# multiplefish/VPLines-SLAM

Hardware: AMD Instinct MI355X
Metric: sliding-window BA solves/sec (10 KF, 200 pts + 80 lines, 5 iters) (higher is better)
Workload: dtype f64

## Files before the change

### vplines-slam_amd/csrc/ba_step.h

```cpp
#pragma once
#include "ba_common.h"
#include "ba_solve.h"

namespace vpl {

constexpr int SCHUR_THREADS = 256;
constexpr int CHOL_THREADS = 256;
constexpr int BACK_THREADS = 256;

__device__ __forceinline__ void lds_ticket_wait(int* t, int seq) {
  while (__hip_atomic_load(t, __ATOMIC_RELAXED, __HIP_MEMORY_SCOPE_WORKGROUP) != seq) __builtin_amdgcn_s_sleep(1);
  __builtin_amdgcn_fence(__ATOMIC_ACQUIRE, "workgroup", "local");
}
__device__ __forceinline__ void lds_ticket_pass(int* t, int seq, int lane) {
  __builtin_amdgcn_fence(__ATOMIC_RELEASE, "workgroup", "local");
  if (lane == 0) __hip_atomic_store(t, seq + 1, __ATOMIC_RELAXED, __HIP_MEMORY_SCOPE_WORKGROUP);
}

__device__ __forceinline__ int compact2vis(int c, int s, int WS) {
  if (c < WS - 6) { const int v = 6 * s + c; return v < 66 ? v : -1; }
  if (c < WS) return 66 + (c - (WS - 6));
  return c < WS + 2 ? 72 + (c - WS) : -1;
}

// ... 253 lines not shown
        const int e = (h0 + u) * T + tid;
        code[u] = (h0 + u < NB && e < NZ_N) ? B.nz_tab[e] : -1;
      }
#pragma unroll
      for (int u = 0; u < HALF; ++u) hh[u] = code[u] >= 0 ? Hcc[code[u] & 0x3fff] : 0.0;
#pragma unroll
      for (int u = 0; u < HALF; ++u)
        if (code[u] >= 0) {
          const int r = (code[u] >> 14) & 255, c = code[u] >> 22;
          qq += (r == c ? 1.0 : 2.0) * uc[r] * hh[u] * uc[c];
        }
    }
  }
  VPL_STAMP(B, w, 1);
  for (int p = tid; p < nP; p += T) {
    const double s = kP[4 * p], d = kP[4 * p + 1], g = kP[4 * p + 2], h = kP[4 * p + 3];
    const double Al = s * s * h + mu * d * d;
    if (!(Al > 0.0)) flag[0] = 1;
    const double smv = s / sqrt(Al);
    pS[p] = smv;
    pE[p] = (s * g / d) / smv;
    pG[p] = smv * (g * d / s);
  }
  for (int l = tid; l < nL; l += T) {
    double Hl[16], s4[4], d4[4], g4[4];
#pragma unroll
    for (int a = 0; a < 4; ++a) { s4[a] = kL[28 * l + a]; d4[a] = kL[28 * l + 4 + a]; g4[a] = kL[28 * l + 8 + a]; }
#pragma unroll
    for (int k = 0; k < 16; ++k) Hl[k] = kL[28 * l + 12 + k];
    double A[10];
    int t = 0;
#pragma unroll
    for (int a = 0; a < 4; ++a)
#pragma unroll
      for (int b = 0; b < 4; ++b) if (b <= a) {
        A[t] = s4[a] * s4[b] * Hl[4 * a + b];
        if (a == b) A[t] += mu * d4[a] * d4[a];
        ++t;
      }
    bool ok = true;
    chol4(A, ok);
    if (!ok) flag[0] = 1;
    double us[4];
#pragma unroll
    for (int k = 0; k < 10; ++k) { lch[l * 10 + k] = A[k]; lC[l * 10 + k] = A[k]; }
#pragma unroll
    for (int a = 0; a < 4; ++a) {
      const double rd = 1.0 / A[tri(a, a)];
      lS[4 * l + a] = s4[a] * rd;
      us[a] = g4[a] / d4[a];
#pragma unroll
      for (int qd = 0; qd < 4; ++qd) if (qd < a) lC[l * 10 + tri(a, qd)] = A[tri(a, qd)] * rd;
    }
#pragma unroll
    for (int a = 0; a < 4; ++a) {
      double s2 = 0;
#pragma unroll
      for (int qd = 0; qd < 4; ++qd) if (qd >= a) s2 += A[tri(qd, a)] * us[qd];
      lE[4 * l + a] = s2;
    }
    {
      double xg[4];
#pragma unroll
      for (int a = 0; a < 4; ++a) {
        double s2 = (s4[a] / A[tri(a, a)]) * (g4[a] * d4[a] / s4[a]);
#pragma unroll
        for (int qd = 0; qd < 4; ++qd) if (qd < a) s2 -= (A[tri(a, qd)] / A[tri(a, a)]) * xg[qd];
        xg[a] = s2;
        lG[4 * l + a] = s2;
      }
    }
  }
  __syncthreads();
  for (int i = tid; i < CSQ_N; i += T) Cacc[i] = 0.0;
  for (int i = tid; i < NLT * 4 * 64; i += T) {
    const int ln = i & 63, v = (i >> 6) & 3, t = i >> 8;
    int ta = 0, tb = 0;
    tri_decode(t, ta, tb);
    const int ca = 16 * ta + (ln >> 4) + 4 * v, cb = 16 * tb + (ln & 15);
    int code = -1;
    if (ca >= cb && ca < WSv + 2 && cb < WSv) {
      const int a0 = compact2vis(ca, 0, WSv), b0 = compact2vis(cb, 0, WSv);
      const int step = (ca < WSv - 6 ? CSQ_LD : 0) + (cb < WSv - 6 ? 1 : 0);
      code = (a0 * CSQ_LD + b0) | step << 16;
    }
    ftab[i] = code;
  }
  __syncthreads();
  VPL_STAMP(B, w, 2);
  {
    const int m = lane & 15, kk = lane >> 4;
    const int wrow = lane < SK_WSTRIDE ? B.sk_wave[((size_t)w * 8 + wv) * SK_WSTRIDE + lane] : -1;
    const int nchunk = __builtin_amdgcn_readlane(wrow, 0);
    auto fetch = [&](int k) {
      int4 e = etab[k];
      e.x = __builtin_amdgcn_readfirstlane(e.x); e.y = __builtin_amdgcn_readfirstlane(e.y); e.z = __builtin_amdgcn_readfirstlane(e.z);
      return e;
    };
    v4d acc[NLT];
#pragma unroll
    for (int t = 0; t < NLT; ++t) acc[t] = v4d{0, 0, 0, 0};
    const double* Wp = B.Wp + (size_t)w * B.maxP * WS;
    const double* Wl = B.Wl + (size_t)w * B.maxL * 4 * WS;
    const double* gpv = B.gp + (size_t)w * B.maxP;
    const double* glv = B.gl + (size_t)w * B.maxL * 4;
    double wm[NTC], gm[NTC], em[NTC];
    int cl[NTC];
#pragma unroll
    for (int t = 0; t < NTC; ++t) {
      const int c = 16 * t + m;
      wm[t] = c < WSv ? 1.0 : 0.0;
      gm[t] = c == WSv ? 1.0 : 0.0;
      em[t] = c == WSv + 1 ? 1.0 : 0.0;
      cl[t] = c < WSv - 6 ? c : (c < WSv ? c + coff : WS - 1);
    }
    auto lm_id = [&](const int4 e) { return ((kk & 2 ? e.z : e.y) >> (16 * (kk & 1))) & 0xffff; };
    auto load_raw = [&](const int4 e, double (&raw)[NTC][4]) {
      const bool isl = (e.x & 32) != 0;
      const int idr = lm_id(e);
      const int id = idr != 0xffff ? idr : 0;
      if (isl) {
        const double* Wr = Wl + (unsigned)(id * 4 * WS);
#pragma unroll
        for (int t = 0; t < NTC; ++t)
#pragma unroll
          for (int qd = 0; qd < 4; ++qd) raw[t][qd] = Wr[(unsigned)(qd * WS + cl[t])];
      } else {
#pragma unroll
        for (int t = 0; t < NTC; ++t) raw[t][0] = Wp[(unsigned)(id * WS + cl[t])];
#pragma unroll
        for (int t = 0; t < NTC; ++t)
#pragma unroll
          for (int qd = 1; qd < 4; ++qd) raw[t][qd] = 0.0;
      }
    };
    auto transform = [&](const int4 e, const double (&raw)[NTC][4], double (&x)[NTC][4]) {
      const bool isl = (e.x & 32) != 0;
      const int idr = lm_id(e);
      const int id = idr != 0xffff ? idr : 0;
      const double pm = idr != 0xffff ? 1.0 : 0.0;
      if (isl) {
        const double* C = lC + id * 10;
        const double s0 = lS[4 * id] * pm, s1 = lS[4 * id + 1] * pm, s2 = lS[4 * id + 2] * pm, s3 = lS[4 * id + 3] * pm;
        const double c10 = C[1], c20 = C[3], c21 = C[4], c30 = C[6], c31 = C[7], c32 = C[8];
        double ev[4], gv[4];
#pragma unroll
        for (int a = 0; a < 4; ++a) { ev[a] = lE[4 * id + a] * pm; gv[a] = lG[4 * id + a] * pm; }
#pragma unroll
        for (int t = 0; t < NTC; ++t) {
          const double x0 = s0 * raw[t][0];
          const double x1 = s1 * raw[t][1] - c10 * x0;
          const double x2 = s2 * raw[t][2] - c20 * x0 - c21 * x1;
          const double x3 = s3 * raw[t][3] - c30 * x0 - c31 * x1 - c32 * x2;
          x[t][0] = x0 * wm[t] + gv[0] * gm[t] + ev[0] * em[t];
          x[t][1] = x1 * wm[t] + gv[1] * gm[t] + ev[1] * em[t];
          x[t][2] = x2 * wm[t] + gv[2] * gm[t] + ev[2] * em[t];
          x[t][3] = x3 * wm[t] + gv[3] * gm[t] + ev[3] * em[t];
        }
      } else {
        const double sp = pS[id] * pm, ep = pE[id] * pm, gq = pG[id] * pm;
#pragma unroll
        for (int t = 0; t < NTC; ++t) {
          x[t][0] = sp * raw[t][0] * wm[t] + gq * gm[t] + ep * em[t];
          x[t][1] = 0.0; x[t][2] = 0.0; x[t][3] = 0.0;
        }
      }
    };
#ifdef VPL_STAMPS
    long long st_flush = 0, st_wait = 0, st_xf = 0, st_mf = 0, st_ld = 0;
#endif
    auto flush = [&](int g, int seq) {
#ifdef VPL_STAMPS
      const long long tf0 = __builtin_readcyclecounter();
#endif
      const int s6 = 6 * (g & 15);
      int code[NLT * 4];
#pragma unroll
      for (int i = 0; i < NLT * 4; ++i) code[i] = ftab[i * 64 + lane];
      lds_ticket_wait(&tick[0], seq);
#ifdef VPL_STAMPS
      st_wait += __builtin_readcyclecounter() - tf0;
#endif
#pragma unroll
      for (int t = 0; t < NLT; ++t) {
        const double vals[4] = {acc[t].x, acc[t].y, acc[t].z, acc[t].w};
#pragma unroll
        for (int v = 0; v < 4; ++v) {
          const int c2 = code[4 * t + v];
          if (c2 >= 0) lds_add(&Cacc[(c2 & 0xffff) + s6 * (c2 >> 16)], vals[v]);
        }
        acc[t] = v4d{0, 0, 0, 0};
      }
      lds_ticket_pass(&tick[0], seq, lane);
#ifdef VPL_STAMPS
      st_flush += __builtin_readcyclecounter() - tf0;
#endif
    };
    int nent = 0;
#pragma unroll 1
    for (int ch = 0; ch < nchunk; ++ch) {
      const int k0 = __builtin_amdgcn_readlane(wrow, __builtin_amdgcn_readfirstlane(1 + 3 * ch));
      const int k1 = __builtin_amdgcn_readlane(wrow, __builtin_amdgcn_readfirstlane(2 + 3 * ch));
      const int seq = __builtin_amdgcn_readlane(wrow, __builtin_amdgcn_readfirstlane(3 + 3 * ch));
      nent += k1 - k0;
      if (MIXED && (fetch(k0).x & 64)) {
        SchurWide A;
        A.etab = etab; A.Wp = Wp; A.Wl = Wl; A.WS = WS; A.lC = lC; A.lS = lS; A.lE = lE; A.lG = lG; A.pS = pS; A.pE = pE; A.pG = pG;
        A.Cacc = Cacc; A.tick = tick;
        schur_wide_chunk(A, k0, k1, seq);
        continue;
      }
      double raw0[NTC][4], raw1[NTC][4], raw2[NTC][4];
      constexpr int NPF = 3;
      load_raw(fetch(k0), raw0);
      load_raw(fetch(min(k0 + 1, k1 - 1)), raw1);
      load_raw(fetch(min(k0 + 2, k1 - 1)), raw2);
      const int gcur = fetch(k0).x;
      auto step = [&](int k, double (&rw)[NTC][4]) {
        const int4 e = fetch(k);
#ifdef VPL_STAMPS
        const long long ts0 = __builtin_readcyclecounter();
#endif
        double x[NTC][4];
        transform(e, rw, x);
#ifdef VPL_STAMPS
        const long long ts1 = __builtin_readcyclecounter();
        st_xf += ts1 - ts0;
#endif
        load_raw(fetch(min(k + NPF, k1 - 1)), rw);
#ifdef VPL_STAMPS
        const long long ts2 = __builtin_readcyclecounter();
        st_ld += ts2 - ts1;
#endif
        const bool isl = (e.x & 32) != 0;
#pragma unroll
        for (int a = 0; a < 4; ++a) {
          if (a == 0 || isl) {
            int t = 0;
#pragma unroll
            for (int ta = 0; ta < NTC; ++ta)
#pragma unroll
              for (int tb = 0; tb <= ta; ++tb, ++t) acc[t] = __builtin_amdgcn_mfma_f64_16x16x4f64(x[ta][a], x[tb][a], acc[t], 0, 0, 0);
          }
        }
#ifdef VPL_STAMPS
        st_mf += __builtin_readcyclecounter() - ts2;
#endif
      };
#pragma unroll 1
      for (int kb = k0; kb < k1; kb += NPF) {
        step(kb, raw0);
        if (kb + 1 < k1) step(kb + 1, raw1);
        if (kb + 2 < k1) step(kb + 2, raw2);
      }
      flush(gcur, seq);
    }
#ifdef VPL_STAMPS
    if (lane == 0 && wv < 2) {
      long long* dg_ = B.dbg + (size_t)w * 64 + 30 + 6 * wv;
      dg_[0] = st_xf; dg_[1] = st_ld; dg_[2] = st_mf; dg_[3] = st_flush; dg_[4] = st_wait; dg_[5] = nent;
    }
#endif
  }
  __syncthreads();
  VPL_STAMP(B, w, 3);
  for (int b = tid; b < NV; b += T) qq += 2.0 * Cacc[(NV + 1) * CSQ_LD + b] * uc[vis2cam(b)];
  double* sacc = B.sacc + (size_t)w * SACC_N;
  for (int i = tid; i < SACC_N; i += T) {
    int a, b;
    tri_decode(i, a, b);
    sacc[i] = Cacc[a * CSQ_LD + b];
  }
  a1 = block_sum(a1, red);
  q = block_sum(q, red);
  qq = block_sum(qq, red);
  if (tid == 0) {
    tr->a1 = a1;
    tr->alpha = a1 / (q + qq);
    if (flag[0]) B.path[w] = 2;
  }
  VPL_STAMP(B, w, 4);
}

template <int NTC>
__global__ __launch_bounds__(SCHUR_THREADS, 2) void k_schur(DevBatch B) {
  extern __shared__ double sm[];
  if (blockIdx.x == 0 && threadIdx.x == 0) { B.ord_cnt[2 * ((B.ord_it + 1) & 1)] = 0; B.ord_cnt[2 * ((B.ord_it + 1) & 1) + 1] = 0; }
  schur_body<NTC>(B, ordered_window(B), sm);
}
__global__ __launch_bounds__(SCHUR_THREADS, 2) void k_schur_mixed(DevBatch B) {
  extern __shared__ double sm[];
  if (blockIdx.x == 0 && threadIdx.x == 0) { B.ord_cnt[2 * ((B.ord_it + 1) & 1)] = 0; B.ord_cnt[2 * ((B.ord_it + 1) & 1) + 1] = 0; }
  schur_body<3, true>(B, ordered_window(B), sm);
}
inline size_t schur_smem(int maxP, int maxL, int ntc = 5) {
  const int r1 = std::max(4 * maxP + 28 * maxL, (int)CSQ_N);
  const int maxKS = maxP / 4 + maxL + NF + 2;
  return (size_t)(r1 + 3 * maxP + 22 * maxL + 176 + 24) * sizeof(double) + (size_t)(8 + 4 * maxKS + ntc * (ntc + 1) / 2 * 256) * sizeof(int);
}

constexpr int DN = 90;
constexpr int DNT = 6;
constexpr int DNAP = DNT * (DNT + 1) / 2 * 256;
#ifdef VPL_CHOL_OCC3
constexpr int XLD = 66;
constexpr int CHOL_MIN_WAVES = 3;
#else
constexpr int XLD = 72;
constexpr int CHOL_MIN_WAVES = 2;
#endif
constexpr int XROWS_A = 36, XROWS_B = 48;

__device__ __forceinline__ int chain_frame(int ch, int b) { return ch == 0 ? 1 + b : 10 - b; }
__device__ __forceinline__ int chain_col(int ch, int b, int lane) {
  if (lane < 18) {
    const int ds = (b & 1) ? 9 : 0;
    const int f = chain_frame(ch, b);
    const int fr = (lane >= ds && lane < ds + 9) ? f : (ch == 0 ? f + 1 : f - 1);
    return 15 * fr + 6 + (lane < 9 ? lane : lane - 9);
  }
  if (ch == 0) {
    if (lane < 27) return 6 + (lane - 18);
    if (lane < 63) return 15 * ((lane - 27) / 6) + (lane - 27) % 6;
    return NC;
  }
  if (lane < 54) return 15 * (5 + (lane - 18) / 6) + (lane - 18) % 6;
  return lane == 54 ? NC : -1;
}
__device__ __forceinline__ int cam2dense(int c) {
  if (c < 0) return -1;
  if (c == NC) return DN;
  const int v = cam2vis(c);
  if (v >= 0) return v;
  if (c < 15) return 72 + (c - 6);
  return (c >= 81 && c < 90) ? c : -1;
}
__device__ __forceinline__ int dense2cam(int d) { return d < NV ? vis2cam(d) : (d < 81 ? 6 + (d - 72) : d); }
__device__ __forceinline__ int chain_dense(int ch, int lane) {
  if (lane < 18) {
    const bool s5 = ch == 0 ? lane < 9 : lane >= 9;
    return s5 ? 81 + (lane < 9 ? lane : lane - 9) : -1;
  }
  return cam2dense(chain_col(ch, 0, lane));
}

__device__ __forceinline__ void chol_body(const DevBatch& B, const int w, double* sm) {
  const int tid = threadIdx.x, T = CHOL_THREADS;
  const int lane = tid & 63, wv = ((tid >> 6) + ((blockIdx.x >> 8) & 1) * 2) & 3;
  TrState* tr = &B.tr[w];
  if (tr->status != 0 || tr->reuse != 0 || B.path[w] != 0) return;
  count_active(B, 1);
  constexpr int REG = (XROWS_A + XROWS_B) * XLD > DNAP ? (XROWS_A + XROWS_B) * XLD : DNAP;
  double* XA = sm;
  double* XBm = sm + XROWS_A * XLD;
  double* S = sm;
  double* scv = sm + REG;
  double* dgv = scv + 176;
  double* ycam = dgv + 176;
  double* yv = ycam + 176;
  double* isd = yv + 96;
  double* Linv = isd + 96;
  double* red = Linv + 256;
  int* flag = (int*)(red + 24);
  int* cdmap = flag + 8;
  double* rsL = (double*)(cdmap + 128);

  const size_t fb = (size_t)w * B.nfull;
  const double* gscale = B.scale + fb;
  const double* gdiag = B.diag + fb;
  const double* ggrad = B.grad + fb;
  double* ggn = B.gn + fb;
  const double* Hcc = B.Hcc + (size_t)w * NCP;
  const double* gc = B.gc + (size_t)w * NC;
  const double* sacc = B.sacc + (size_t)w * SACC_N;
  const double mu = tr->mu;
  for (int c = tid; c < 176; c += T) { scv[c] = c < NC ? gscale[c] : 0.0; dgv[c] = c < NC ? gdiag[c] : 1.0; ycam[c] = 0.0; }
  if (tid < 4) flag[tid] = 0;
  if (tid < 128) cdmap[tid] = chain_dense(tid >> 6, tid & 63);
  for (int i = tid; i < 3 * XLD; i += T) XBm[(XROWS_B - 3) * XLD + i] = 0.0;
  __syncthreads();
  VPL_STAMP(B, w, 8);

  double U[45];
#pragma unroll
  for (int i = 0; i < 45; ++i) U[i] = 0.0;
#define Xs(b, k) U[9 * (b) + (k)]
  if (wv < 2) {
    const int ch = wv, nblk = ch == 0 ? 4 : 5;
    double* Xout = ch == 0 ? XA : XBm;
    bool bad = false;
    auto load_strip = [&](int b, double (&raw)[9]) {
      const int col = chain_col(ch, b, lane);
      const int f = chain_frame(ch, b);
#pragma unroll
      for (int i = 0; i < 9; ++i) {
        const int r = 15 * f + 6 + i;
        raw[i] = 0.0;
        if (col == NC) raw[i] = gc[r];
        else if (col >= 0) raw[i] = Hcc[col > r ? tri(col, r) : tri(r, col)];
      }
    };
    double rawn[9];
    load_strip(0, rawn);
#pragma unroll
    for (int b = 0; b < 5; ++b) {
      if (b < nblk) {
        const int ds = (b & 1) ? 9 : 0, ns = 9 - ds;
        const int col = chain_col(ch, b, lane);
        const int f = chain_frame(ch, b);
        double R[9];
        {
          const double scol = col == NC ? 1.0 : (col >= 0 ? scv[col] : 0.0);
#pragma unroll
          for (int i = 0; i < 9; ++i) {
            const int r = 15 * f + 6 + i;
            R[i] = rawn[i] * (scv[r] * scol);
            if (col == r) R[i] += mu * dgv[r] * dgv[r];
          }
        }
        if (b + 1 < nblk) load_strip(b + 1, rawn);
        if (b > 0) {
          const bool fresh = lane >= ns && lane < ns + 9;
#pragma unroll
          for (int k = 0; k < 9; ++k) {
            const double xk = fresh ? 0.0 : Xs(b - 1, k);
#pragma unroll
            for (int i = 0; i < 9; ++i) R[i] -= readlane_f64(Xs(b - 1, k), ds + i) * xk;
          }
        }
        double piv[9];
#pragma unroll
        for (int k = 0; k < 9; ++k) {
          const double pk = readlane_f64(R[k], ds + k);
          piv[k] = pk;
          if (!(pk > 0.0)) bad = true;
          double rinv = __builtin_amdgcn_rcp(pk);
          rinv = fma(rinv, fma(-pk, rinv, 1.0), rinv);
          rinv = fma(rinv, fma(-pk, rinv, 1.0), rinv);
          const double fj = R[k] * rinv;
#pragma unroll
          for (int i = k + 1; i < 9; ++i) R[i] -= readlane_f64(R[i], ds + k) * fj;
        }
        const bool dcol = cam2dense(col) >= 0;
#pragma unroll
        for (int k = 0; k < 9; ++k) {
          double rs = __builtin_amdgcn_rsq(piv[k]);
          rs = rs * fma(-0.5 * piv[k] * rs, rs, 1.5);
          rs = rs * fma(-0.5 * piv[k] * rs, rs, 1.5);
          if (lane == 0) rsL[(5 * ch + b) * 9 + k] = rs;
          const double xv = R[k] * rs;
          Xs(b, k) = col >= 0 ? xv : 0.0;
          Xout[(9 * b + k) * XLD + lane] = dcol ? xv : 0.0;
        }
        __builtin_amdgcn_fence(__ATOMIC_RELEASE, "workgroup");
        if (lane == 0) __hip_atomic_store(&flag[1 + ch], b + 1, __ATOMIC_RELAXED, __HIP_MEMORY_SCOPE_WORKGROUP);
      }
    }
    if (bad && lane == 0) flag[0] = 1;
  } else {
    const int ch = wv - 2, nblk = ch == 0 ? 4 : 5;
    const double* Xin = ch == 0 ? XA : XBm;
    const int m = lane & 15, kk = lane >> 4;
    const int nks = (ch == 0 ? XROWS_A : XROWS_B) / 4;
    int have = 0;
    v4d pacc[10];
#pragma unroll
    for (int t = 0; t < 10; ++t) pacc[t] = v4d{0, 0, 0, 0};
    for (int ks = 0; ks < nks; ++ks) {
      const int need = min(nblk, (4 * ks + 3) / 9 + 1);
      while (have < need) {
        have = __hip_atomic_load(&flag[1 + ch], __ATOMIC_RELAXED, __HIP_MEMORY_SCOPE_WORKGROUP);
        if (have >= need) __builtin_amdgcn_fence(__ATOMIC_ACQUIRE, "workgroup");
      }
      const double* row = Xin + (4 * ks + kk) * XLD + m;
      const double x0 = row[0], x1 = row[16], x2 = row[32], x3 = row[48];
      pacc[0] = __builtin_amdgcn_mfma_f64_16x16x4f64(x0, x0, pacc[0], 0, 0, 0);
      pacc[1] = __builtin_amdgcn_mfma_f64_16x16x4f64(x1, x0, pacc[1], 0, 0, 0);
      pacc[2] = __builtin_amdgcn_mfma_f64_16x16x4f64(x1, x1, pacc[2], 0, 0, 0);
      pacc[3] = __builtin_amdgcn_mfma_f64_16x16x4f64(x2, x0, pacc[3], 0, 0, 0);
      pacc[4] = __builtin_amdgcn_mfma_f64_16x16x4f64(x2, x1, pacc[4], 0, 0, 0);
      pacc[5] = __builtin_amdgcn_mfma_f64_16x16x4f64(x2, x2, pacc[5], 0, 0, 0);
      pacc[6] = __builtin_amdgcn_mfma_f64_16x16x4f64(x3, x0, pacc[6], 0, 0, 0);
      pacc[7] = __builtin_amdgcn_mfma_f64_16x16x4f64(x3, x1, pacc[7], 0, 0, 0);
      pacc[8] = __builtin_amdgcn_mfma_f64_16x16x4f64(x3, x2, pacc[8], 0, 0, 0);
      pacc[9] = __builtin_amdgcn_mfma_f64_16x16x4f64(x3, x3, pacc[9], 0, 0, 0);
    }
#pragma unroll
    for (int t = 0; t < 10; ++t) { U[4 * t] = pacc[t].x; U[4 * t + 1] = pacc[t].y; U[4 * t + 2] = pacc[t].z; U[4 * t + 3] = pacc[t].w; }
  }
  __syncthreads();
  VPL_STAMP(B, w, 9);

  auto put = [&](int r, int c, double v) {
    S[tix(r, c)] = v;
    if ((r >> 4) == (c >> 4) && r != c) S[tix(c, r)] = v;
  };
  {
    constexpr int NVP = NV * (NV + 1) / 2;
    constexpr int NB1 = (NVP + CHOL_THREADS - 1) / CHOL_THREADS;
    constexpr int NB2 = (19 * 96 + CHOL_THREADS - 1) / CHOL_THREADS;
    double hh[NB1], ss[NB1], h2[NB2], s2[NB2];
    int rc1[NB1], rc2[NB2];
#pragma unroll
    for (int u = 0; u < NB1; ++u) {
      const int e = u * T + tid;
      hh[u] = 0.0; ss[u] = 0.0; rc1[u] = -1;
      if (e < NVP) {
        int vr, vc;
        tri_decode(e, vr, vc);
        rc1[u] = vr | vc << 8;
        hh[u] = Hcc[tri(vis2cam(vr), vis2cam(vc))];
        ss[u] = sacc[e];
      }
    }
#pragma unroll
    for (int u = 0; u < NB2; ++u) {
      const int idx = u * T + tid;
      const int i = idx / 96, dc = idx - 96 * i;
      const int dr = 72 + i;
      h2[u] = 0.0; s2[u] = 0.0; rc2[u] = -1;
      if (idx < 19 * 96 && dc <= dr && dc < DN) {
        rc2[u] = dr | dc << 8;
        const int c = dense2cam(dc);
        if (dr < DN) {
          const int r = dense2cam(dr);
          h2[u] = Hcc[r >= c ? tri(r, c) : tri(c, r)];
        } else {
          h2[u] = gc[c];
          if (dc < NV) s2[u] = sacc[tri(NV, dc)];
        }
      }
    }
    for (int i = tid; i < DNAP; i += T) S[i] = 0.0;
    __syncthreads();
    VPL_STAMP(B, w, 14);
#pragma unroll
    for (int u = 0; u < NB1; ++u)
      if (rc1[u] >= 0) {
        const int vr = rc1[u] & 255, vc = rc1[u] >> 8;
        const int r = vis2cam(vr), c = vis2cam(vc);
        double v = (hh[u] - ss[u]) * (scv[r] * scv[c]);
        if (r == c) v += mu * dgv[r] * dgv[r];
        put(vr, vc, v);
      }
#pragma unroll
    for (int u = 0; u < NB2; ++u)
      if (rc2[u] >= 0) {
        const int dr = rc2[u] & 255, dc = rc2[u] >> 8;
        const int c = dense2cam(dc);
        if (dr < DN) {
          const int r = dense2cam(dr);
          double v = h2[u] * (scv[r] * scv[c]);
          if (r == c) v += mu * dgv[r] * dgv[r];
          put(dr, dc, v);
        } else {
          put(DN, dc, (h2[u] - s2[u]) * scv[c]);
        }
      }
    if (tid < 6) S[tix(DN + tid, DN + tid)] = 1.0;
  }
  __syncthreads();
  VPL_STAMP(B, w, 15);
  auto in_both = [](int d) { return (d >= 30 && d < 36) || d >= 81; };
#pragma unroll 1
  for (int pass = 0; pass < 2; ++pass) {
    if ((wv == 2 && pass == 0) || wv == 3) {
      const int ch = wv - 2;
      const int m = lane & 15, kk = lane >> 4;
      int t = 0;
#pragma unroll
      for (int ta = 0; ta < 4; ++ta)
#pragma unroll
        for (int tb = 0; tb <= ta; ++tb, ++t) {
          const int j = 16 * tb + m, dj = cdmap[64 * ch + j];
#pragma unroll
          for (int v = 0; v < 4; ++v) {
            const int i = 16 * ta + kk + 4 * v;
            if (i < j) continue;
            const int di = cdmap[64 * ch + i];
            if (di < 0 || dj < 0) continue;
            if (ch == 1 && (in_both(di) && in_both(dj)) != (pass == 1)) continue;
            const int r = di > dj ? di : dj, c = di > dj ? dj : di;
            if (c >= DN) continue;
            const double val = U[4 * t + v];
            S[tix(r, c)] -= val;
            if ((r >> 4) == (c >> 4) && r != c) S[tix(c, r)] -= val;
          }
        }
    }
    __syncthreads();
  }
  VPL_STAMP(B, w, 10);

  {
    constexpr int NWV = CHOL_THREADS / 64;
    for (int K = 0; K < DNT; ++K) {
      auto rank_update = [&](int col, int I, int J0, int J1) {
        const int m = lane & 15, kk = lane >> 4;
        double* Ct = S + ((I * (I + 1) / 2 + col) << 8);
        v4d c;
        c.x = Ct[tsw(kk, m)]; c.y = Ct[tsw(kk + 4, m)]; c.z = Ct[tsw(kk + 8, m)]; c.w = Ct[tsw(kk + 12, m)];
        for (int J = J0; J < J1; ++J) {
          const double* Ai = S + ((I * (I + 1) / 2 + J) << 8);
          const double* Bk = S + ((col * (col + 1) / 2 + J) << 8);
#pragma unroll
          for (int ks = 0; ks < 4; ++ks) {
            const double av = -Ai[tsw(m, 4 * ks + kk)];
            const double bv = Bk[tsw(m, 4 * ks + kk)];
            c = __builtin_amdgcn_mfma_f64_16x16x4f64(av, bv, c, 0, 0, 0);
          }
        }
        Ct[tsw(kk, m)] = c.x; Ct[tsw(kk + 4, m)] = c.y; Ct[tsw(kk + 8, m)] = c.z; Ct[tsw(kk + 12, m)] = c.w;
      };
      if (wv == 0) {
        double* D = S + ((K * (K + 1) / 2 + K) << 8);
        const int r4 = lane >> 4, cc = lane & 15;
        double d[4], mm[4];
#pragma unroll
        for (int v = 0; v < 4; ++v) { d[v] = D[tsw(r4 + 4 * v, cc)]; mm[v] = (r4 + 4 * v == cc) ? 1.0 : 0.0; }
        const int ncol = min(16, DN - 16 * K);
        double pivc = 1.0;
        bool bad = false;
#define VPL_DSTEP(J) diag_tile_step<J>(d, mm, r4, cc, ncol, pivc, bad);
        VPL_DSTEP(0) VPL_DSTEP(1) VPL_DSTEP(2) VPL_DSTEP(3) VPL_DSTEP(4) VPL_DSTEP(5) VPL_DSTEP(6) VPL_DSTEP(7)
        VPL_DSTEP(8) VPL_DSTEP(9) VPL_DSTEP(10) VPL_DSTEP(11) VPL_DSTEP(12) VPL_DSTEP(13) VPL_DSTEP(14) VPL_DSTEP(15)
#undef VPL_DSTEP
        if (bad) {
          if (lane == 0) flag[0] = 1;
        } else {
          const double sq = sqrt(pivc);
          if (cc < ncol) {
#pragma unroll
            for (int v = 0; v < 4; ++v) {
              const int r = r4 + 4 * v;
              if (r > cc) D[tsw(r, cc)] = d[v] / sq;
              else if (r == cc) { const double id = 1.0 / sq; isd[16 * K + cc] = id; D[tsw(r, cc)] = 1.0 / id; }
            }
          }
          if (K < DNT - 1) {
            const double isq = 1.0 / sq;
#pragma unroll
            for (int v = 0; v < 4; ++v) {
              const int r = r4 + 4 * v;
              const double ir = __shfl(isq, r, 64);
              Linv[tsw(r, cc)] = cc <= r ? mm[v] * ir : 0.0;
            }
          }
        }
      } else if (K >= 1) {
        for (int I = K + 1 + (wv - 1); I < DNT; I += NWV - 1) rank_update(K, I, K - 1, K);
        if (K + 1 < DNT)
          for (int I = K + 1 + (wv - 1); I < DNT; I += NWV - 1) rank_update(K + 1, I, 0, K);
      }
      __syncthreads();
      if (flag[0]) break;
      for (int I = K + 1 + wv; I < DNT; I += NWV) {
        const int m = lane & 15, kk = lane >> 4;
        double* At = S + ((I * (I + 1) / 2 + K) << 8);
        v4d c = {0.0, 0.0, 0.0, 0.0};
        double av[4], bv[4];
#pragma unroll
        for (int ks = 0; ks < 4; ++ks) { av[ks] = At[tsw(m, 4 * ks + kk)]; bv[ks] = Linv[tsw(m, 4 * ks + kk)]; }
#pragma unroll
        for (int ks = 0; ks < 4; ++ks) c = __builtin_amdgcn_mfma_f64_16x16x4f64(av[ks], bv[ks], c, 0, 0, 0);
        At[tsw(kk, m)] = c.x; At[tsw(kk + 4, m)] = c.y; At[tsw(kk + 8, m)] = c.z; At[tsw(kk + 12, m)] = c.w;
        if (I == K + 1) {
          __builtin_amdgcn_fence(__ATOMIC_RELEASE, "workgroup");
          __builtin_amdgcn_wave_barrier();
          __builtin_amdgcn_fence(__ATOMIC_ACQUIRE, "workgroup");
          rank_update(K + 1, K + 1, K, K + 1);
        }
      }
      __syncthreads();
    }
  }
  __syncthreads();
  if (flag[0]) {
    if (tid == 0) B.path[w] = 2;
    return;
  }
  VPL_STAMP(B, w, 11);
  for (int c = tid; c < 96; c += T) yv[c] = c < DN ? S[tix(DN, c)] : 0.0;
  __syncthreads();
  for (int K = DNT - 1; K >= 0; --K) {
    const double* D = S + ((K * (K + 1) / 2 + K) << 8);
    if (wv == 0) {
      const int ncol = min(16, DN - 16 * K);
      double yl = lane < 16 ? yv[16 * K + lane] : 0.0;
      const double isdl = lane < ncol ? isd[16 * K + lane] : 0.0;
      double Lcol[16];
#pragma unroll
      for (int j = 0; j < 16; ++j) Lcol[j] = (lane < j && j < ncol) ? D[tsw(j, lane & 15)] : 0.0;
#pragma unroll
      for (int j = 15; j >= 0; --j) {
        if (j < ncol) {
          const double yj = readlane_f64(yl, j) * readlane_f64(isdl, j);
          if (lane < j) yl -= Lcol[j] * yj;
          if (lane == j) yl = yj;
        }
      }
      if (lane < ncol) yv[16 * K + lane] = yl;
    }
    __syncthreads();
    for (int c = tid; c < 16 * K; c += T) {
      const double* Lk = S + ((K * (K + 1) / 2 + (c >> 4)) << 8);
      double s2 = 0.0;
#pragma unroll
      for (int r = 0; r < 16; ++r) s2 += Lk[tsw(r, c & 15)] * yv[16 * K + r];
      yv[c] -= s2;
    }
    __syncthreads();
  }
  for (int d = tid; d < DN; d += T) ycam[dense2cam(d)] = yv[d];
  __syncthreads();
  VPL_STAMP(B, w, 12);
  if (wv < 2) {
    const int ch = wv, nblk = ch == 0 ? 4 : 5;
#pragma unroll
    for (int b = 4; b >= 0; --b) {
      if (b < nblk) {
        const int ds = (b & 1) ? 9 : 0;
        const int col = chain_col(ch, b, lane);
        const int f = chain_frame(ch, b);
        const bool pivl = lane >= ds && lane < ds + 9;
        const double cf = col == NC ? 1.0 : ((col < 0 || pivl) ? 0.0 : -ycam[col]);
        double t[9];
#pragma unroll
        for (int k = 0; k < 9; ++k) t[k] = wave_sum_dpp(Xs(b, k) * cf);
#pragma unroll
        for (int j = 8; j >= 0; --j) {
          const double yj = t[j] * rsL[(5 * ch + b) * 9 + j];
#pragma unroll
          for (int k = 0; k < j; ++k) t[k] -= readlane_f64(Xs(b, k), ds + j) * yj;
          t[j] = yj;
        }
        if (lane == 0) {
#pragma unroll
          for (int j = 0; j < 9; ++j) ycam[15 * f + 6 + j] = t[j];
        }
        __builtin_amdgcn_fence(__ATOMIC_RELEASE, "workgroup");
        __builtin_amdgcn_wave_barrier();
        __builtin_amdgcn_fence(__ATOMIC_ACQUIRE, "workgroup");
      }
    }
  }
  __syncthreads();
  double a2 = 0.0, a3 = 0.0;
  double* ycs = B.ycs + (size_t)w * 176;
  for (int c = tid; c < 176; c += T) {
    double u = 0.0;
    if (c < NC) {
      const double y = ycam[c];
      u = scv[c] * y;
      const double gnv = -dgv[c] * y;
      ggn[c] = gnv;
      a2 += gnv * gnv;
      a3 += ggrad[c] * gnv;
    }
    ycs[c] = u;
  }
  a2 = block_sum(a2, red);
  a3 = block_sum(a3, red);
  if (tid == 0) { B.sx[(size_t)w * 8] = a2; B.sx[(size_t)w * 8 + 1] = a3; }
  VPL_STAMP(B, w, 13);
}
#undef Xs
__global__ __launch_bounds__(CHOL_THREADS, CHOL_MIN_WAVES) void k_chol(DevBatch B) {
  extern __shared__ double sm[];
  chol_body(B, ordered_window(B), sm);
}
constexpr size_t CHOL_SMEM = (size_t)(((XROWS_A + XROWS_B) * XLD > DNAP ? (XROWS_A + XROWS_B) * XLD : DNAP) + 3 * 176 + 2 * 96 + 256 + 24 + 96) * sizeof(double) + (8 + 128) * sizeof(int);

__device__ __forceinline__ void back_body(const DevBatch& B, const int w, double* sm) {
  const int tid = threadIdx.x, T = BACK_THREADS;
  const int lane = tid & 63;
  TrState* tr = &B.tr[w];
  if (tr->status != 0) return;
  const int path = B.path[w];
  if (path != 0) {
    __syncthreads();
    if (tid == 0 && path == 2) B.path[w] = 0;
    return;
  }
  const int nP = B.nP[w], nL = B.nL[w];
  const int WS = B.WS;
  double* uc = sm;
  double* lrhs = uc + 176;
  double* lgn = lrhs + 4 * B.maxL;
  double* gdelta = lgn + B.nfull;
  double* red = gdelta + B.nfull;
  int* pSt = (int*)(red + 24);
  int* lSt = pSt + B.maxP;
  const size_t fb = (size_t)w * B.nfull;
  const double* gscale = B.scale + fb;
  const double* gdiag = B.diag + fb;
  const double* ggrad = B.grad + fb;
  double* ggn = B.gn + fb;
  const double* lch = B.lchol + (size_t)w * B.maxL * 10;
  const int LP = NC, LL = NC + B.maxP;
  const bool reuse0 = tr->reuse != 0;
  count_active(B, reuse0 ? 2 : 1);
  VPL_STAMP(B, w, 5);
  if (!reuse0) {
    const double mu = tr->mu;
    for (int p = tid; p < nP; p += T) pSt[p] = B.pt_start[(size_t)w * B.maxP + p];
    for (int l = tid; l < nL; l += T) lSt[l] = B.ln_start[(size_t)w * B.maxL + l];
    for (int c = tid; c < 176; c += T) uc[c] = c < NV ? B.ycs[(size_t)w * 176 + vis2cam(c)] : 0.0;
    for (int c = tid; c < NC; c += T) lgn[c] = ggn[c];
    __syncthreads();
    double a2 = 0.0, a3 = 0.0;
    {
      const int sub = lane & 7, grp = tid >> 3;
      const int nblk = WS / 6;
      constexpr int NPH = 4;
      for (int p0 = 0; p0 < nP; p0 += NPH * (T / 8)) {
        double wyv[NPH], sv[NPH], dv[NPH], hv[NPH], gv2[NPH], grv[NPH];
        size_t piv[NPH];
#pragma unroll
        for (int h = 0; h < NPH; ++h) {
          const int p = p0 + h * (T / 8) + grp;
          piv[h] = (size_t)w * B.maxP + (p < nP ? p : 0);
          wyv[h] = 0.0; sv[h] = dv[h] = 1.0; hv[h] = gv2[h] = grv[h] = 0.0;
          if (p < nP) {
            const int s0 = pSt[p];
            for (int blk = sub; blk < nblk; blk += 8) {
              const bool exb = blk == nblk - 1;
              const int vb = exb ? 66 : 6 * (s0 + blk);
              if (!exb && vb >= 66) continue;
              const double* Wr = B.Wp + piv[h] * WS + 6 * blk;
#pragma unroll
              for (int k = 0; k < 6; ++k) wyv[h] += Wr[k] * uc[vb + k];
            }
            if (sub == 0) {
              sv[h] = gscale[LP + p]; dv[h] = gdiag[LP + p]; hv[h] = B.Hpp[piv[h]]; gv2[h] = B.gp[piv[h]];
              grv[h] = ggrad[LP + p];
            }
          }
        }
#pragma unroll
        for (int h = 0; h < NPH; ++h) {
          const int p = p0 + h * (T / 8) + grp;
          double wy = wyv[h];
          wy += __shfl_xor(wy, 1, 64); wy += __shfl_xor(wy, 2, 64); wy += __shfl_xor(wy, 4, 64);
          if (p < nP && sub == 0) {
            const double s = sv[h], d = dv[h];
            const double Al = s * s * hv[h] + mu * d * d;
            const double y = s * (gv2[h] - wy) / Al;
            const double gnv = -d * y;
            ggn[LP + p] = gnv; lgn[LP + p] = gnv;
            a2 += gnv * gnv;
            a3 += grv[h] * gnv;
          }
        }
      }
      constexpr int NLH = 5;
      for (int r0 = 0; r0 < 4 * nL; r0 += NLH * (T / 8)) {
        double wyv[NLH], glv[NLH];
#pragma unroll
        for (int h = 0; h < NLH; ++h) {
          const int r = r0 + h * (T / 8) + grp, l = r >> 2, a = r & 3;
          wyv[h] = 0.0; glv[h] = 0.0;
          if (l < nL) {
            const size_t li = (size_t)w * B.maxL + l;
            const int s0 = lSt[l];
            for (int blk = sub; blk < nblk; blk += 8) {
              const bool exb = blk == nblk - 1;
              const int vb = exb ? 66 : 6 * (s0 + blk);
              if (!exb && vb >= 66) continue;
              const double* Wr = B.Wl + (li * 4 + a) * WS + 6 * blk;
#pragma unroll
              for (int k = 0; k < 6; ++k) wyv[h] += Wr[k] * uc[vb + k];
            }
            if (sub == 0) glv[h] = B.gl[li * 4 + a];
          }
        }
#pragma unroll
        for (int h = 0; h < NLH; ++h) {
          const int r = r0 + h * (T / 8) + grp;
          double wy = wyv[h];
          wy += __shfl_xor(wy, 1, 64); wy += __shfl_xor(wy, 2, 64); wy += __shfl_xor(wy, 4, 64);
          if (r < 4 * nL && sub == 0) lrhs[r] = gscale[LL + r] * (glv[h] - wy);
        }
      }
      __syncthreads();
      for (int l = tid; l < nL; l += T) {
        double C[10], t4[4], gd4[4], gr4[4];
#pragma unroll
        for (int k = 0; k < 10; ++k) C[k] = lch[l * 10 + k];
#pragma unroll
        for (int k = 0; k < 4; ++k) { gd4[k] = gdiag[LL + 4 * l + k]; gr4[k] = ggrad[LL + 4 * l + k]; }
#pragma unroll
        for (int k = 0; k < 4; ++k) t4[k] = lrhs[4 * l + k];
#pragma unroll
        for (int k = 0; k < 4; ++k) {
// ... 141 lines not shown
```

Before: 254,200.

## Build reduced camera matrix directly in dense tile layout via MFMA accumulators

Chain strips are now written into the X buffers at dense-tile column positions, so the MFMA syrk produces contributions already aligned to the 6x6 dense tile grid. The two consumer waves split the 21 tiles by parity, fold the H0 assembly (Hcc minus sacc, scaling, damping) into the accumulators, and write final tiles straight into S. This removes the separate scatter-assembly phase, the cdmap table and the two-pass scatter-subtract with its extra barriers. In exchange it zero-fills the whole X region and computes h0 element-wise with scattered global reads per tile, and each consumer wave now processes both chains serially.

Result: faster. 260,300, median of 6 (+2.4%).

```diff
diff --git a/vplines-slam_amd/csrc/ba_step.h b/vplines-slam_amd/csrc/ba_step.h
--- a/vplines-slam_amd/csrc/ba_step.h
+++ b/vplines-slam_amd/csrc/ba_step.h
@@ -579,14 +579,11 @@
 constexpr int DN = 90;
 constexpr int DNT = 6;
 constexpr int DNAP = DNT * (DNT + 1) / 2 * 256;
-#ifdef VPL_CHOL_OCC3
-constexpr int XLD = 66;
-constexpr int CHOL_MIN_WAVES = 3;
-#else
-constexpr int XLD = 72;
+constexpr int XLD = 80;
 constexpr int CHOL_MIN_WAVES = 2;
-#endif
 constexpr int XROWS_A = 36, XROWS_B = 48;
+__device__ __forceinline__ constexpr int xcol(int ch, int J) { return ch == 0 ? 16 * (J > 3 ? J - 1 : J) : 16 * (J - 1); }
+__device__ __forceinline__ constexpr int tile_row(int t) { return t < 1 ? 0 : t < 3 ? 1 : t < 6 ? 2 : t < 10 ? 3 : t < 15 ? 4 : 5; }
 
 __device__ __forceinline__ int chain_frame(int ch, int b) { return ch == 0 ? 1 + b : 10 - b; }
 __device__ __forceinline__ int chain_col(int ch, int b, int lane) {
@@ -639,8 +636,7 @@
   double* Linv = isd + 96;
   double* red = Linv + 256;
   int* flag = (int*)(red + 24);
-  int* cdmap = flag + 8;
-  double* rsL = (double*)(cdmap + 128);
+  double* rsL = (double*)(flag + 8);
 
   const size_t fb = (size_t)w * B.nfull;
   const double* gscale = B.scale + fb;
@@ -653,8 +649,7 @@
   const double mu = tr->mu;
   for (int c = tid; c < 176; c += T) { scv[c] = c < NC ? gscale[c] : 0.0; dgv[c] = c < NC ? gdiag[c] : 1.0; ycam[c] = 0.0; }
   if (tid < 4) flag[tid] = 0;
-  if (tid < 128) cdmap[tid] = chain_dense(tid >> 6, tid & 63);
-  for (int i = tid; i < 3 * XLD; i += T) XBm[(XROWS_B - 3) * XLD + i] = 0.0;
+  for (int i = tid; i < (XROWS_A + XROWS_B) * XLD; i += T) sm[i] = 0.0;
   __syncthreads();
   VPL_STAMP(B, w, 8);
 
@@ -665,6 +660,8 @@
   if (wv < 2) {
     const int ch = wv, nblk = ch == 0 ? 4 : 5;
     double* Xout = ch == 0 ? XA : XBm;
+    const int xd = chain_dense(ch, lane);
+    const int xp = xd < 0 ? -1 : xcol(ch, xd >> 4) + (xd & 15);
     bool bad = false;
     auto load_strip = [&](int b, double (&raw)[9]) {
       const int col = chain_col(ch, b, lane);
@@ -727,7 +724,7 @@
           if (lane == 0) rsL[(5 * ch + b) * 9 + k] = rs;
           const double xv = R[k] * rs;
           Xs(b, k) = col >= 0 ? xv : 0.0;
-          Xout[(9 * b + k) * XLD + lane] = dcol ? xv : 0.0;
+          if (xp >= 0) Xout[(9 * b + k) * XLD + xp] = dcol ? xv : 0.0;
         }
         __builtin_amdgcn_fence(__ATOMIC_RELEASE, "workgroup");
         if (lane == 0) __hip_atomic_store(&flag[1 + ch], b + 1, __ATOMIC_RELAXED, __HIP_MEMORY_SCOPE_WORKGROUP);
@@ -735,138 +732,95 @@
     }
     if (bad && lane == 0) flag[0] = 1;
   } else {
-    const int ch = wv - 2, nblk = ch == 0 ? 4 : 5;
-    const double* Xin = ch == 0 ? XA : XBm;
     const int m = lane & 15, kk = lane >> 4;
-    const int nks = (ch == 0 ? XROWS_A : XROWS_B) / 4;
+    auto h0 = [&](int r, int c) -> double {
+      if (r < c) { const int t = r; r = c; c = t; }
+      if (r > DN || c == DN) return r == c ? 1.0 : 0.0;
+      const int cc = dense2cam(c);
+      if (r == DN) return (gc[cc] - (c < NV ? sacc[tri(NV, c)] : 0.0)) * scv[cc];
+      const int cr = dense2cam(r);
+      double v = Hcc[cr >= cc ? tri(cr, cc) : tri(cc, cr)];
+      if (r < NV) v -= sacc[tri(r, c)];
+      v *= scv[cr] * scv[cc];
+      if (r == c) v += mu * dgv[cr] * dgv[cr];
+      return v;
+    };
+    const int p = __builtin_amdgcn_readfirstlane(wv - 2);
+    v4d hs[11], acc[11];
+#pragma unroll
+    for (int i = 0; i < 11; ++i) acc[i] = v4d{0, 0, 0, 0};
     int have = 0;
-    v4d pacc[10];
-#pragma unroll
-    for (int t = 0; t < 10; ++t) pacc[t] = v4d{0, 0, 0, 0};
-    for (int ks = 0; ks < nks; ++ks) {
-      const int need = min(nblk, (4 * ks + 3) / 9 + 1);
+#pragma unroll 1
+    for (int ks = 0; ks < XROWS_A / 4; ++ks) {
+      const int need = min(4, (4 * ks + 3) / 9 + 1);
       while (have < need) {
-        have = __hip_atomic_load(&flag[1 + ch], __ATOMIC_RELAXED, __HIP_MEMORY_SCOPE_WORKGROUP);
+        have = __hip_atomic_load(&flag[1], __ATOMIC_RELAXED, __HIP_MEMORY_SCOPE_WORKGROUP);
         if (have >= need) __builtin_amdgcn_fence(__ATOMIC_ACQUIRE, "workgroup");
       }
-      const double* row = Xin + (4 * ks + kk) * XLD + m;
-      const double x0 = row[0], x1 = row[16], x2 = row[32], x3 = row[48];
-      pacc[0] = __builtin_amdgcn_mfma_f64_16x16x4f64(x0, x0, pacc[0], 0, 0, 0);
-      pacc[1] = __builtin_amdgcn_mfma_f64_16x16x4f64(x1, x0, pacc[1], 0, 0, 0);
-      pacc[2] = __builtin_amdgcn_mfma_f64_16x16x4f64(x1, x1, pacc[2], 0, 0, 0);
-      pacc[3] = __builtin_amdgcn_mfma_f64_16x16x4f64(x2, x0, pacc[3], 0, 0, 0);
-      pacc[4] = __builtin_amdgcn_mfma_f64_16x16x4f64(x2, x1, pacc[4], 0, 0, 0);
-      pacc[5] = __builtin_amdgcn_mfma_f64_16x16x4f64(x2, x2, pacc[5], 0, 0, 0);
-      pacc[6] = __builtin_amdgcn_mfma_f64_16x16x4f64(x3, x0, pacc[6], 0, 0, 0);
-      pacc[7] = __builtin_amdgcn_mfma_f64_16x16x4f64(x3, x1, pacc[7], 0, 0, 0);
-      pacc[8] = __builtin_amdgcn_mfma_f64_16x16x4f64(x3, x2, pacc[8], 0, 0, 0);
-      pacc[9] = __builtin_amdgcn_mfma_f64_16x16x4f64(x3, x3, pacc[9], 0, 0, 0);
-    }
-#pragma unroll
-    for (int t = 0; t < 10; ++t) { U[4 * t] = pacc[t].x; U[4 * t + 1] = pacc[t].y; U[4 * t + 2] = pacc[t].z; U[4 * t + 3] = pacc[t].w; }
+      const double* row = XA + (4 * ks + kk) * XLD + m;
+      double x[6];
+#pragma unroll
+      for (int J = 0; J < 6; ++J) x[J] = J == 3 ? 0.0 : row[xcol(0, J)];
+#pragma unroll
+      for (int t = 0; t < 21; ++t) {
+        const int I = tile_row(t), J = t - I * (I + 1) / 2;
+        if ((t & 1) != p || I == 3 || J == 3) continue;
+        acc[t >> 1] = __builtin_amdgcn_mfma_f64_16x16x4f64(x[I], x[J], acc[t >> 1], 0, 0, 0);
+      }
+    }
+#pragma unroll
+    for (int t = 0; t < 21; ++t) {
+      if ((t & 1) != p) continue;
+      const int I = tile_row(t), J = t - I * (I + 1) / 2;
+      const int r = 16 * I + kk, c = 16 * J + m;
+      const v4d h = v4d{h0(r, c), h0(r + 4, c), h0(r + 8, c), h0(r + 12, c)};
+      hs[t >> 1] = (I == 3 || J == 3) ? h : h - acc[t >> 1];
+      acc[t >> 1] = v4d{0, 0, 0, 0};
+    }
+    if (p) hs[10] = v4d{0, 0, 0, 0};
+    have = 0;
+#pragma unroll 1
+    for (int ks = 0; ks < XROWS_B / 4; ++ks) {
+      const int need = min(5, (4 * ks + 3) / 9 + 1);
+      while (have < need) {
+        have = __hip_atomic_load(&flag[2], __ATOMIC_RELAXED, __HIP_MEMORY_SCOPE_WORKGROUP);
+        if (have >= need) __builtin_amdgcn_fence(__ATOMIC_ACQUIRE, "workgroup");
+      }
+      const double* row = XBm + (4 * ks + kk) * XLD + m;
+      double x[6];
+#pragma unroll
+      for (int J = 0; J < 6; ++J) x[J] = J == 0 ? 0.0 : row[xcol(1, J)];
+#pragma unroll
+      for (int t = 0; t < 21; ++t) {
+        const int I = tile_row(t), J = t - I * (I + 1) / 2;
+        if ((t & 1) != p || J == 0) continue;
+        acc[t >> 1] = __builtin_amdgcn_mfma_f64_16x16x4f64(x[I], x[J], acc[t >> 1], 0, 0, 0);
+      }
+    }
+#pragma unroll
+    for (int i = 0; i < 11; ++i) {
+      const v4d h = hs[i] - acc[i];
+      U[4 * i] = h.x; U[4 * i + 1] = h.y; U[4 * i + 2] = h.z; U[4 * i + 3] = h.w;
+    }
   }
   __syncthreads();
   VPL_STAMP(B, w, 9);
 
-  auto put = [&](int r, int c, double v) {
-    S[tix(r, c)] = v;
-    if ((r >> 4) == (c >> 4) && r != c) S[tix(c, r)] = v;
-  };
-  {
-    constexpr int NVP = NV * (NV + 1) / 2;
-    constexpr int NB1 = (NVP + CHOL_THREADS - 1) / CHOL_THREADS;
-    constexpr int NB2 = (19 * 96 + CHOL_THREADS - 1) / CHOL_THREADS;
-    double hh[NB1], ss[NB1], h2[NB2], s2[NB2];
-    int rc1[NB1], rc2[NB2];
-#pragma unroll
-    for (int u = 0; u < NB1; ++u) {
-      const int e = u * T + tid;
-      hh[u] = 0.0; ss[u] = 0.0; rc1[u] = -1;
-      if (e < NVP) {
-        int vr, vc;
-        tri_decode(e, vr, vc);
-        rc1[u] = vr | vc << 8;
-        hh[u] = Hcc[tri(vis2cam(vr), vis2cam(vc))];
-        ss[u] = sacc[e];
-      }
-    }
-#pragma unroll
-    for (int u = 0; u < NB2; ++u) {
-      const int idx = u * T + tid;
-      const int i = idx / 96, dc = idx - 96 * i;
-      const int dr = 72 + i;
-      h2[u] = 0.0; s2[u] = 0.0; rc2[u] = -1;
-      if (idx < 19 * 96 && dc <= dr && dc < DN) {
-        rc2[u] = dr | dc << 8;
-        const int c = dense2cam(dc);
-        if (dr < DN) {
-          const int r = dense2cam(dr);
-          h2[u] = Hcc[r >= c ? tri(r, c) : tri(c, r)];
-        } else {
-          h2[u] = gc[c];
-          if (dc < NV) s2[u] = sacc[tri(NV, dc)];
-        }
-      }
-    }
-    for (int i = tid; i < DNAP; i += T) S[i] = 0.0;
-    __syncthreads();
-    VPL_STAMP(B, w, 14);
-#pragma unroll
-    for (int u = 0; u < NB1; ++u)
-      if (rc1[u] >= 0) {
-        const int vr = rc1[u] & 255, vc = rc1[u] >> 8;
-        const int r = vis2cam(vr), c = vis2cam(vc);
-        double v = (hh[u] - ss[u]) * (scv[r] * scv[c]);
-        if (r == c) v += mu * dgv[r] * dgv[r];
-        put(vr, vc, v);
-      }
-#pragma unroll
-    for (int u = 0; u < NB2; ++u)
-      if (rc2[u] >= 0) {
-        const int dr = rc2[u] & 255, dc = rc2[u] >> 8;
-        const int c = dense2cam(dc);
-        if (dr < DN) {
-          const int r = dense2cam(dr);
-          double v = h2[u] * (scv[r] * scv[c]);
-          if (r == c) v += mu * dgv[r] * dgv[r];
-          put(dr, dc, v);
-        } else {
-          put(DN, dc, (h2[u] - s2[u]) * scv[c]);
-        }
-      }
-    if (tid < 6) S[tix(DN + tid, DN + tid)] = 1.0;
+  if (wv >= 2) {
+    const int p = __builtin_amdgcn_readfirstlane(wv - 2);
+    const int m = lane & 15, kk = lane >> 4;
+#pragma unroll
+    for (int t = 0; t < 21; ++t) {
+      if ((t & 1) != p) continue;
+      double* St = S + (t << 8);
+#pragma unroll
+      for (int v = 0; v < 4; ++v) {
+        const int r = kk + 4 * v;
+        St[tsw(r, m)] = (t == 20 && r == DN - 80 && m == DN - 80) ? 1.0 : U[4 * (t >> 1) + v];
+      }
+    }
   }
   __syncthreads();
-  VPL_STAMP(B, w, 15);
-  auto in_both = [](int d) { return (d >= 30 && d < 36) || d >= 81; };
-#pragma unroll 1
-  for (int pass = 0; pass < 2; ++pass) {
-    if ((wv == 2 && pass == 0) || wv == 3) {
-      const int ch = wv - 2;
-      const int m = lane & 15, kk = lane >> 4;
-      int t = 0;
-#pragma unroll
-      for (int ta = 0; ta < 4; ++ta)
-#pragma unroll
-        for (int tb = 0; tb <= ta; ++tb, ++t) {
-          const int j = 16 * tb + m, dj = cdmap[64 * ch + j];
-#pragma unroll
-          for (int v = 0; v < 4; ++v) {
-            const int i = 16 * ta + kk + 4 * v;
-            if (i < j) continue;
-            const int di = cdmap[64 * ch + i];
-            if (di < 0 || dj < 0) continue;
-            if (ch == 1 && (in_both(di) && in_both(dj)) != (pass == 1)) continue;
-            const int r = di > dj ? di : dj, c = di > dj ? dj : di;
-            if (c >= DN) continue;
-            const double val = U[4 * t + v];
-            S[tix(r, c)] -= val;
-            if ((r >> 4) == (c >> 4) && r != c) S[tix(c, r)] -= val;
-          }
-        }
-    }
-    __syncthreads();
-  }
   VPL_STAMP(B, w, 10);
 
   {
```
